# zhiqiangdon/pose-adv-aug

Hardware: AMD Instinct MI355X
Metric: images/sec, 2-stack HG 256x256 bs=24 per GPU, full training step (higher is better)
Workload: dtype bf16; 1 GPU; BASELINE configs[1]: 2-stack hourglass chan 256, bs=24/GPU, 256x256 MPII-shape synthetic frames (720x1280 uint8 resident in HBM), on-device HumanAug warp, heat-map MSE, RMSprop, PCKh; global_batch=24, parallelism=dp1, ranks_seen=1, devices_seen=1

## Files before the change

### pose_adv_aug_amd/csrc/crop_warp.hip

```cpp
#include "pose_ops.h"

#pragma clang fp contract(off)

#define CW_PREC 22

struct CropPlan {
    int wb, hb;
    int case_b;
    int wd, hd;
    int ulx, uly;
    int nw, nh;
    int cw, ch;
    int pad, rot_mode;
    int dx0, dx1, dy0, dy1;
    int sy0, sy1;
    int sx0, sx1;
    int flip;
    float gain[3];
    double m[6];
    double sx, sy;
};

__device__ __forceinline__ int src_byte(unsigned char k, float gain, bool f32) {
    float v = ((float)k / 255.f) * gain;
    v = fminf(fmaxf(v, 0.f), 1.f);
    if (f32) { const float t = v * 255.f; return (int)(t + 0.5f); }
    return (int)((double)v * 255.0 + 0.5);
}

#define CW_ACC 12
#define CW_TAB 768
// ... 40 lines not shown
    if (xmin < 0) xmin = 0;
    int xmax = (int)(t.center + support + 0.5);
    if (xmax > in_size) xmax = in_size;
    t.xmin = xmin; t.n = xmax - xmin;
    double ww = 0.0;
    for (int x = 0; x < t.n; ++x) {
        double v = ((double)(x + xmin) - t.center + 0.5) * t.ss;
        if (v < 0.0) v = -v;
        ww += v < 1.0 ? 1.0 - v : 0.0;
    }
    t.ww = ww;
    return t;
}
__device__ __forceinline__ int tap_coeff(const Taps& t, int x) {
    double v = ((double)(x + t.xmin) - t.center + 0.5) * t.ss;
    if (v < 0.0) v = -v;
    double w = v < 1.0 ? 1.0 - v : 0.0;
    if (t.ww != 0.0) w = w / t.ww;
    return (int)(0.5 + w * (double)(1 << CW_PREC));
}
__device__ __forceinline__ int clip8(int ss) { ss >>= CW_PREC; return ss < 0 ? 0 : (ss > 255 ? 255 : ss); }

#define CW_KMAX 24
#define CW_ENTRY (2 + CW_KMAX)
__device__ __forceinline__ const int* tap_entry(const int* table, int b, int axis, int axis_max, int i) {
    return table + (((size_t)b * 4 + axis) * axis_max + i) * CW_ENTRY;
}

__global__ void crop_plan_kernel(const double* params, const int* sizes, int Hs, int Ws, int B, int res, CropPlan* plans, unsigned* acc) {
    const int b = blockIdx.x * blockDim.x + threadIdx.x;
    if (b >= B) return;
    if (acc)
        for (int i = 0; i < CW_ACC; ++i) acc[(size_t)b * CW_ACC + i] = (i % 6) < 3 ? 255u : 0u;
    const double* p = params + (size_t)b * 8;
    CropPlan P;
    P.wb = sizes ? sizes[2 * b] : Ws; P.hb = sizes ? sizes[2 * b + 1] : Hs;
    P.flip = p[4] != 0.0;
    for (int c = 0; c < 3; ++c) P.gain[c] = (float)p[5 + c];
    float cx = (float)p[0], cy = (float)p[1], s = (float)p[2];
    const double rot = p[3];
    double sf = (double)(s * 200.f) / (double)res;
    P.case_b = sf >= 2.0;
    if (!P.case_b) sf = 1.0;
    P.wd = P.wb; P.hd = P.hb; P.sx = P.sy = 1.0;
    if (P.case_b) {
        const double frac = 1.0 / sf;
// ... 18 lines not shown
    P.ulx = ulx; P.uly = uly; P.nw = brx - ulx; P.nh = bry - uly;
    for (int i = 0; i < 6; ++i) P.m[i] = 0.0;
    if (rot != 0.0) {
        double angle = fmod(rot, 360.0);
        if (angle < 0.0) angle += 360.0;
        if (angle == 0.0) P.rot_mode = 0;
        else if (angle == 180.0) P.rot_mode = 2;
        else if ((angle == 90.0 || angle == 270.0) && P.nw == P.nh) P.rot_mode = angle == 90.0 ? 3 : 4;
        else {
            P.rot_mode = 1;
            const double ar = -(angle * (3.14159265358979323846 / 180.0));
            const double cs = cos(ar), sn = sin(ar);
            const double rcx = (double)P.nw / 2.0, rcy = (double)P.nh / 2.0;
            P.m[0] = cs; P.m[1] = sn; P.m[3] = -sn; P.m[4] = cs;
            P.m[2] = (P.m[0] * (-rcx) + P.m[1] * (-rcy) + 0.0) + rcx;
            P.m[5] = (P.m[3] * (-rcx) + P.m[4] * (-rcy) + 0.0) + rcy;
        }
    }
    P.dx0 = ulx < 0 ? 0 : ulx; P.dx1 = brx < P.wd ? brx : P.wd;
    P.dy0 = uly < 0 ? 0 : uly; P.dy1 = bry < P.hd ? bry : P.hd;
    if (P.dx1 < P.dx0) P.dx1 = P.dx0;
    if (P.dy1 < P.dy0) P.dy1 = P.dy0;
    P.sy0 = 0; P.sy1 = 0; P.sx0 = 0; P.sx1 = 0;
    if (P.case_b && P.dy1 > P.dy0) {
        const Taps t0 = taps_of(P.dy0, P.hb, P.sy), t1 = taps_of(P.dy1 - 1, P.hb, P.sy);
        P.sy0 = t0.xmin; P.sy1 = t1.xmin + t1.n;
    }
    if (P.case_b && P.dx1 > P.dx0) {
        const Taps t0 = taps_of(P.dx0, P.wb, P.sx), t1 = taps_of(P.dx1 - 1, P.wb, P.sx);
        P.sx0 = t0.xmin; P.sx1 = t1.xmin + t1.n;
    }
    plans[b] = P;
}

__global__ void crop_coeff_kernel(const CropPlan* plans, int res, int* table, int axis_max) {
    const CropPlan& P = plans[blockIdx.y];
    const int axis = blockIdx.z;
    int count, first, in_size; double scale;
    if (axis == 0) { if (!P.case_b) return; count = P.dx1 - P.dx0; first = P.dx0; in_size = P.wb; scale = P.sx; }
    else if (axis == 1) { if (!P.case_b) return; count = P.dy1 - P.dy0; first = P.dy0; in_size = P.hb; scale = P.sy; }
    else if (axis == 2) { if (P.cw == res) return; count = res; first = 0; in_size = P.cw; scale = (double)P.cw / (double)res; }
    else { if (P.ch == res) return; count = res; first = 0; in_size = P.ch; scale = (double)P.ch / (double)res; }
    const int i = blockIdx.x * blockDim.x + threadIdx.x;
    if (i >= count || i >= axis_max) return;
    const Taps t = taps_of(first + i, in_size, scale);
    int* e = table + (((size_t)blockIdx.y * 4 + axis) * axis_max + i) * CW_ENTRY;
    e[0] = t.xmin;
    if (t.n > CW_KMAX) { e[1] = -t.n; return; }
    e[1] = t.n;
    for (int k = 0; k < t.n; ++k) e[2 + k] = tap_coeff(t, k);
}

template <bool STRETCH>
__global__ __launch_bounds__(256) void crop_src_kernel(const unsigned char* src, int Hs, int Ws, const CropPlan* plans, uchar4* s4, size_t s4_stride,
                                                       int s4_pitch, const unsigned* acc) {
    const CropPlan& P = plans[blockIdx.y];
    if (!P.case_b) return;
    const int ncol = P.sx1 - P.sx0, nrow = P.sy1 - P.sy0;
    const unsigned char* img = src + (size_t)blockIdx.y * Hs * Ws * 3;
    uchar4* out = s4 + (size_t)blockIdx.y * s4_stride;
    __shared__ unsigned char lut[3][256];
    if (STRETCH) {
        float lo, hi;
        stretch_range(acc + (size_t)blockIdx.y * CW_ACC, acc + (size_t)blockIdx.y * CW_ACC + 3, P.gain, false, false, lo, hi);
        for (int k = threadIdx.x; k < 768; k += blockDim.x) lut[k >> 8][k & 255] = stretch_f32(src_val((unsigned char)(k & 255), P.gain[k >> 8]), lo, hi);
    } else
        for (int k = threadIdx.x; k < 768; k += blockDim.x) lut[k >> 8][k & 255] = (unsigned char)src_byte((unsigned char)(k & 255), P.gain[k >> 8], true);
    __syncthreads();
    if ((Ws & 3) == 0 && ((size_t)src & 3) == 0) {
        const int lo = P.flip ? P.wb - P.sx1 : P.sx0, hi = lo + ncol;
        const int g0 = lo >> 2, ng = ((hi - 1) >> 2) - g0 + 1;
        const unsigned total = (unsigned)ng * (unsigned)nrow;
        for (unsigned i = blockIdx.x * blockDim.x + threadIdx.x; i < total; i += gridDim.x * blockDim.x) {
            const unsigned r = i / (unsigned)ng, g = i - r * (unsigned)ng;
            const int c0 = (g0 + (int)g) << 2;
            const unsigned* w = reinterpret_cast<const unsigned*>(img + ((size_t)(P.sy0 + (int)r) * Ws + c0) * 3);
            const unsigned w0 = w[0], w1 = w[1], w2 = w[2];
            const unsigned char b[12] = {(unsigned char)w0, (unsigned char)(w0 >> 8), (unsigned char)(w0 >> 16), (unsigned char)(w0 >> 24),
                                         (unsigned char)w1, (unsigned char)(w1 >> 8), (unsigned char)(w1 >> 16), (unsigned char)(w1 >> 24),
                                         (unsigned char)w2, (unsigned char)(w2 >> 8), (unsigned char)(w2 >> 16), (unsigned char)(w2 >> 24)};
            uchar4* orow = out + (size_t)r * s4_pitch;
#pragma unroll
            for (int k = 0; k < 4; ++k) {
                const int cs = c0 + k;
                if (cs < lo || cs >= hi) continue;
                const int x = (P.flip ? P.wb - 1 - cs : cs) - P.sx0;
                orow[x] = make_uchar4(lut[0][b[3 * k]], lut[1][b[3 * k + 1]], lut[2][b[3 * k + 2]], 0);
            }
        }
        return;
    }
    const long total = (long)ncol * nrow;
    for (long i = (long)blockIdx.x * blockDim.x + threadIdx.x; i < total; i += (long)gridDim.x * blockDim.x) {
        const int r = (int)(i / ncol), x = (int)(i - (long)r * ncol);
        const int xs = P.sx0 + x;
        const unsigned char* px = img + ((size_t)(P.sy0 + r) * Ws + (P.flip ? P.wb - 1 - xs : xs)) * 3;
        out[(size_t)r * s4_pitch + x] = make_uchar4(lut[0][px[0]], lut[1][px[1]], lut[2][px[2]], 0);
    }
}

#define CW_HREG 12
#define CW_HROWS 16
template <int NT>
__device__ __forceinline__ void down_h_rows(const uchar4* col, int s4_pitch, uchar4* out, int t1_pitch, int xc, int r0, int nrow, const int* e, int n) {
    int w[NT];
#pragma unroll
    for (int k = 0; k < NT; ++k) w[k] = k < n ? e[2 + k] : 0;
#pragma unroll 2
    for (int j = 0; j < CW_HROWS; ++j) {
        const int r = r0 + 4 * j;
        if (r >= nrow) break;
        const uchar4* row = col + (size_t)r * s4_pitch;
        int a0 = 1 << (CW_PREC - 1), a1 = a0, a2 = a0;
#pragma unroll
        for (int k = 0; k < NT; ++k) {
            const uchar4 px = row[k];
            a0 += (int)px.x * w[k]; a1 += (int)px.y * w[k]; a2 += (int)px.z * w[k];
        }
        out[(size_t)r * t1_pitch + xc] = make_uchar4((unsigned char)clip8(a0), (unsigned char)clip8(a1), (unsigned char)clip8(a2), 0);
    }
}

__global__ __launch_bounds__(256) void crop_down_h_kernel(const CropPlan* plans, const int* table, int axis_max, const uchar4* s4, size_t s4_stride,
                                                          int s4_pitch, uchar4* t1, size_t t1_stride, int t1_pitch, int col_blocks) {
    const CropPlan& P = plans[blockIdx.y];
    if (!P.case_b) return;
    const int ncol = P.dx1 - P.dx0, nrow = P.sy1 - P.sy0;
    const int cb = blockIdx.x % col_blocks, rb = blockIdx.x / col_blocks;
    const int xc = cb * 64 + (threadIdx.x & 63);
    const int r0 = rb * (4 * CW_HROWS) + (threadIdx.x >> 6);
    if (xc >= ncol || r0 >= nrow) return;
    const uchar4* in = s4 + (size_t)blockIdx.y * s4_stride;
    uchar4* out = t1 + (size_t)blockIdx.y * t1_stride;
    const int* e = tap_entry(table, blockIdx.y, 0, axis_max, xc);
    const int xmin = e[0], n = e[1];
    if (n >= 0 && n <= CW_HREG) {
        if (n <= 8) down_h_rows<8>(in + (xmin - P.sx0), s4_pitch, out, t1_pitch, xc, r0, nrow, e, n);
        else down_h_rows<CW_HREG>(in + (xmin - P.sx0), s4_pitch, out, t1_pitch, xc, r0, nrow, e, n);
        return;
    }
    for (int j = 0; j < CW_HROWS; ++j) {
        const int r = r0 + 4 * j;
        if (r >= nrow) break;
        int a0 = 1 << (CW_PREC - 1), a1 = a0, a2 = a0;
        if (n >= 0) {
            const uchar4* row = in + (size_t)r * s4_pitch + (xmin - P.sx0);
            for (int k = 0; k < n; ++k) {
                const uchar4 px = row[k];
                const int w = e[2 + k];
                a0 += (int)px.x * w; a1 += (int)px.y * w; a2 += (int)px.z * w;
            }
        } else {
            const Taps t = taps_of(P.dx0 + xc, P.wb, P.sx);
            const uchar4* row = in + (size_t)r * s4_pitch + (t.xmin - P.sx0);
            for (int k = 0; k < t.n; ++k) {
                const uchar4 px = row[k];
                const int w = tap_coeff(t, k);
                a0 += (int)px.x * w; a1 += (int)px.y * w; a2 += (int)px.z * w;
            }
        }
        out[(size_t)r * t1_pitch + xc] = make_uchar4((unsigned char)clip8(a0), (unsigned char)clip8(a1), (unsigned char)clip8(a2), 0);
    }
}

__global__ void crop_down_v_kernel(const CropPlan* plans, const int* table, int axis_max, const uchar4* t1, size_t t1_stride, int t1_pitch,
                                   uchar4* d, size_t d_stride, int d_pitch) {
    const CropPlan& P = plans[blockIdx.y];
    if (!P.case_b) return;
    const int ncol = P.dx1 - P.dx0, nrow = P.dy1 - P.dy0;
    const long total = (long)ncol * nrow;
    const uchar4* in = t1 + (size_t)blockIdx.y * t1_stride;
    uchar4* out = d + (size_t)blockIdx.y * d_stride;
    for (long i = (long)blockIdx.x * blockDim.x + threadIdx.x; i < total; i += (long)gridDim.x * blockDim.x) {
        const int yr = (int)(i / ncol), xc = (int)(i - (long)yr * ncol);
        const int* e = tap_entry(table, blockIdx.y, 1, axis_max, yr);
        int a0 = 1 << (CW_PREC - 1), a1 = a0, a2 = a0;
        if (e[1] >= 0) {
            const int ymin = e[0], n = e[1];
            for (int k = 0; k < n; ++k) {
                const uchar4 px = in[(size_t)(ymin + k - P.sy0) * t1_pitch + xc];
                const int w = e[2 + k];
                a0 += (int)px.x * w; a1 += (int)px.y * w; a2 += (int)px.z * w;
            }
        } else {
            const Taps t = taps_of(P.dy0 + yr, P.hb, P.sy);
            for (int k = 0; k < t.n; ++k) {
                const uchar4 px = in[(size_t)(t.xmin + k - P.sy0) * t1_pitch + xc];
                const int w = tap_coeff(t, k);
                a0 += (int)px.x * w; a1 += (int)px.y * w; a2 += (int)px.z * w;
            }
        }
        out[(size_t)yr * d_pitch + xc] = make_uchar4((unsigned char)clip8(a0), (unsigned char)clip8(a1), (unsigned char)clip8(a2), 0);
    }
}

__device__ __forceinline__ void minmax_commit(unsigned (&mn)[3], unsigned (&mx)[3], unsigned* a) {
    __shared__ unsigned red[6];
    if (threadIdx.x < 6) red[threadIdx.x] = threadIdx.x < 3 ? 255u : 0u;
    __syncthreads();
#pragma unroll
    for (int c = 0; c < 3; ++c)
        for (int o = 32; o > 0; o >>= 1) {
            const unsigned n = (unsigned)__shfl_xor((int)mn[c], o, 64), x = (unsigned)__shfl_xor((int)mx[c], o, 64);
            mn[c] = n < mn[c] ? n : mn[c]; mx[c] = x > mx[c] ? x : mx[c];
        }
    if ((threadIdx.x & 63) == 0)
        for (int c = 0; c < 3; ++c) { atomicMin(&red[c], mn[c]); atomicMax(&red[3 + c], mx[c]); }
    __syncthreads();
    if (threadIdx.x < 3) atomicMin(&a[threadIdx.x], red[threadIdx.x]);
    else if (threadIdx.x < 6) atomicMax(&a[threadIdx.x], red[threadIdx.x]);
}

__global__ __launch_bounds__(256) void crop_minmax_src_kernel(const unsigned char* src, int Hs, int Ws, const CropPlan* plans, unsigned* acc) {
    const CropPlan& P = plans[blockIdx.y];
    int x0 = 0, x1 = P.wb, y0 = 0, y1 = P.hb;
    unsigned* a = acc + (size_t)blockIdx.y * CW_ACC;
// ... 44 lines not shown
    for (unsigned i = blockIdx.x * blockDim.x + threadIdx.x; i < total; i += gridDim.x * blockDim.x) {
        const unsigned yr = i / (unsigned)ncol, xc = i - yr * (unsigned)ncol;
        const uchar4 px = in[(size_t)yr * d_pitch + xc];
        const unsigned v[3] = {px.x, px.y, px.z};
#pragma unroll
        for (int c = 0; c < 3; ++c) { mn[c] = v[c] < mn[c] ? v[c] : mn[c]; mx[c] = v[c] > mx[c] ? v[c] : mx[c]; }
    }
    minmax_commit(mn, mx, acc + (size_t)blockIdx.y * CW_ACC + 6);
}

__global__ __launch_bounds__(256) void crop_stretch_table_kernel(const CropPlan* plans, const unsigned* acc, unsigned char* tabs) {
    const CropPlan& P = plans[blockIdx.x];
    const unsigned* a = acc + (size_t)blockIdx.x * CW_ACC + 6;
    const bool zero = P.ulx < 0 || P.uly < 0 || P.ulx + P.nw > P.wd || P.uly + P.nh > P.hd;
    float lo, hi;
    stretch_range(a, a + 3, P.gain, P.case_b != 0, zero, lo, hi);
    const unsigned char k = (unsigned char)threadIdx.x;
    unsigned char* tab = tabs + (size_t)blockIdx.x * CW_TAB;
    for (int c = 0; c < 3; ++c)
        tab[c * 256 + k] = stretch_f64(P.case_b ? (double)k : (double)src_val(k, P.gain[c]), (double)lo, (double)hi);
}

template <bool STRETCH>
__device__ __forceinline__ void window_px(const CropPlan& P, const unsigned char* img, int Ws, const uchar4* d, int d_pitch, const unsigned char* tab,
                                          int yy, int xx, int (&v)[3]) {
    const int gx = P.ulx + xx, gy = P.uly + yy;
    v[0] = v[1] = v[2] = 0;
    if (gx < 0 || gy < 0 || gx >= P.wd || gy >= P.hd) return;
    if (P.case_b) {
        const uchar4 px = d[(size_t)(gy - P.dy0) * d_pitch + (gx - P.dx0)];
        if (STRETCH) { v[0] = tab[px.x]; v[1] = tab[256 + px.y]; v[2] = tab[512 + px.z]; }
        else { v[0] = px.x; v[1] = px.y; v[2] = px.z; }
    } else {
        const unsigned char* px = img + ((size_t)gy * Ws + (P.flip ? P.wb - 1 - gx : gx)) * 3;
        if (STRETCH) { v[0] = tab[px[0]]; v[1] = tab[256 + px[1]]; v[2] = tab[512 + px[2]]; }
        else { v[0] = src_byte(px[0], P.gain[0], false); v[1] = src_byte(px[1], P.gain[1], false); v[2] = src_byte(px[2], P.gain[2], false); }
    }
}

template <bool STRETCH>
__global__ void crop_rotate_kernel(const unsigned char* src, int Hs, int Ws, const CropPlan* plans, const uchar4* d, size_t d_stride, int d_pitch,
                                   uchar4* u, size_t u_stride, int u_pitch, const unsigned char* tabs) {
    const CropPlan& P = plans[blockIdx.y];
    if (P.rot_mode == 0) return;
    const unsigned char* tab = STRETCH ? tabs + (size_t)blockIdx.y * CW_TAB : nullptr;
    const long total = (long)P.cw * P.ch;
    const unsigned char* img = src + (size_t)blockIdx.y * Hs * Ws * 3;
    const uchar4* dd = d + (size_t)blockIdx.y * d_stride;
    uchar4* out = u + (size_t)blockIdx.y * u_stride;
    for (long i = (long)blockIdx.x * blockDim.x + threadIdx.x; i < total; i += (long)gridDim.x * blockDim.x) {
        const int y = (int)(i / P.cw), x = (int)(i - (long)y * P.cw);
        const int X = x + P.pad, Y = y + P.pad;
        int o[3] = {0, 0, 0};
        if (P.rot_mode == 2) window_px<STRETCH>(P, img, Ws, dd, d_pitch, tab, P.nh - 1 - Y, P.nw - 1 - X, o);
        else if (P.rot_mode == 3) window_px<STRETCH>(P, img, Ws, dd, d_pitch, tab, X, P.nw - 1 - Y, o);
        else if (P.rot_mode == 4) window_px<STRETCH>(P, img, Ws, dd, d_pitch, tab, P.nh - 1 - X, Y, o);
        else {
            const double xc = (double)X + 0.5, yc = (double)Y + 0.5;
            double xin = P.m[0] * xc + P.m[1] * yc + P.m[2];
            double yin = P.m[3] * xc + P.m[4] * yc + P.m[5];
            if (!(xin < 0.0 || xin >= (double)P.nw || yin < 0.0 || yin >= (double)P.nh)) {
                xin -= 0.5; yin -= 0.5;
                const int fx = (int)floor(xin), fy = (int)floor(yin);
                const double ddx = xin - (double)fx, ddy = yin - (double)fy;
                const int x0 = fx < 0 ? 0 : (fx < P.nw ? fx : P.nw - 1), x1 = fx + 1 < 0 ? 0 : (fx + 1 < P.nw ? fx + 1 : P.nw - 1);
                const int y0 = fy < 0 ? 0 : (fy < P.nh ? fy : P.nh - 1);
                int p00[3], p01[3], p10[3], p11[3];
                window_px<STRETCH>(P, img, Ws, dd, d_pitch, tab, y0, x0, p00); window_px<STRETCH>(P, img, Ws, dd, d_pitch, tab, y0, x1, p01);
// ... 4 lines not shown
                    const double v2 = has1 ? (double)p10[c] + (double)(p11[c] - p10[c]) * ddx : v1;
                    o[c] = (int)(unsigned char)(v1 + (v2 - v1) * ddy);
                }
            }
        }
        out[(size_t)y * u_pitch + x] = make_uchar4((unsigned char)o[0], (unsigned char)o[1], (unsigned char)o[2], 0);
    }
}

template <bool STRETCH>
__device__ __forceinline__ void crop_px(const CropPlan& P, const unsigned char* img, int Ws, const uchar4* d, int d_pitch, const unsigned char* tab,
                                        const uchar4* u, int u_pitch, int y, int x, int (&v)[3]) {
    if (P.rot_mode != 0) { const uchar4 px = u[(size_t)y * u_pitch + x]; v[0] = px.x; v[1] = px.y; v[2] = px.z; return; }
    const int off = (P.nw - P.cw) / 2;
    window_px<STRETCH>(P, img, Ws, d, d_pitch, tab, y + off, x + off, v);
}

template <bool STRETCH>
__global__ void crop_resize_h_kernel(const unsigned char* src, int Hs, int Ws, const CropPlan* plans, const uchar4* d, size_t d_stride, int d_pitch,
                                     const uchar4* u, size_t u_stride, int u_pitch, int res, const int* table, int axis_max, uchar4* t2, size_t t2_stride,
                                     const unsigned char* tabs) {
    const CropPlan& P = plans[blockIdx.y];
    if (P.cw == res && P.ch == res) return;
    const unsigned char* tab = STRETCH ? tabs + (size_t)blockIdx.y * CW_TAB : nullptr;
    const long total = (long)P.ch * res;
    const unsigned char* img = src + (size_t)blockIdx.y * Hs * Ws * 3;
    const uchar4* dd = d + (size_t)blockIdx.y * d_stride;
    const uchar4* uu = u + (size_t)blockIdx.y * u_stride;
    uchar4* out = t2 + (size_t)blockIdx.y * t2_stride;
    const double scale = (double)P.cw / (double)res;
    for (long i = (long)blockIdx.x * blockDim.x + threadIdx.x; i < total; i += (long)gridDim.x * blockDim.x) {
        const int y = (int)(i / res), uo = (int)(i - (long)y * res);
        int v[3];
        if (P.cw == res) {
            crop_px<STRETCH>(P, img, Ws, dd, d_pitch, tab, uu, u_pitch, y, uo, v);
        } else {
            const int* e = tap_entry(table, blockIdx.y, 2, axis_max, uo);
            int a0 = 1 << (CW_PREC - 1), a1 = a0, a2 = a0;
            if (e[1] >= 0) {
                const int xmin = e[0], n = e[1];
                for (int k = 0; k < n; ++k) {
                    int px[3];
                    crop_px<STRETCH>(P, img, Ws, dd, d_pitch, tab, uu, u_pitch, y, xmin + k, px);
                    const int w = e[2 + k];
                    a0 += px[0] * w; a1 += px[1] * w; a2 += px[2] * w;
                }
            } else {
                const Taps t = taps_of(uo, P.cw, scale);
                for (int k = 0; k < t.n; ++k) {
                    int px[3];
                    crop_px<STRETCH>(P, img, Ws, dd, d_pitch, tab, uu, u_pitch, y, t.xmin + k, px);
                    const int w = tap_coeff(t, k);
                    a0 += px[0] * w; a1 += px[1] * w; a2 += px[2] * w;
                }
            }
            v[0] = clip8(a0); v[1] = clip8(a1); v[2] = clip8(a2);
        }
        out[(size_t)y * res + uo] = make_uchar4((unsigned char)v[0], (unsigned char)v[1], (unsigned char)v[2], 0);
    }
}

template <bool STRETCH>
__global__ void crop_resize_v_kernel(const unsigned char* src, int Hs, int Ws, const CropPlan* plans, const uchar4* d, size_t d_stride, int d_pitch,
                                     const uchar4* u, size_t u_stride, int u_pitch, const uchar4* t2, size_t t2_stride, int res,
                                     const int* table, int axis_max, bf16* out4, float* outf, unsigned char* out8, const unsigned char* tabs) {
    const CropPlan& P = plans[blockIdx.y];
    const int b = blockIdx.y;
    const unsigned char* tab = STRETCH ? tabs + (size_t)b * CW_TAB : nullptr;
    const long total = (long)res * res;
    const unsigned char* img = src + (size_t)b * Hs * Ws * 3;
    const uchar4* dd = d + (size_t)b * d_stride;
    const uchar4* uu = u + (size_t)b * u_stride;
    const uchar4* tt = t2 + (size_t)b * t2_stride;
    const double scale = (double)P.ch / (double)res;
    for (long i = (long)blockIdx.x * blockDim.x + threadIdx.x; i < total; i += (long)gridDim.x * blockDim.x) {
        const int vo = (int)(i / res), uo = (int)(i - (long)vo * res);
        int v[3];
        if (P.cw == res && P.ch == res) {
            crop_px<STRETCH>(P, img, Ws, dd, d_pitch, tab, uu, u_pitch, vo, uo, v);
        } else if (P.ch == res) {
            const uchar4 px = tt[(size_t)vo * res + uo]; v[0] = px.x; v[1] = px.y; v[2] = px.z;
        } else {
            const int* e = tap_entry(table, b, 3, axis_max, vo);
            int a0 = 1 << (CW_PREC - 1), a1 = a0, a2 = a0;
            if (e[1] >= 0) {
                const int ymin = e[0], n = e[1];
                for (int k = 0; k < n; ++k) {
                    const uchar4 px = tt[(size_t)(ymin + k) * res + uo];
                    const int w = e[2 + k];
                    a0 += (int)px.x * w; a1 += (int)px.y * w; a2 += (int)px.z * w;
                }
            } else {
                const Taps t = taps_of(vo, P.ch, scale);
                for (int k = 0; k < t.n; ++k) {
                    const uchar4 px = tt[(size_t)(t.xmin + k) * res + uo];
                    const int w = tap_coeff(t, k);
                    a0 += (int)px.x * w; a1 += (int)px.y * w; a2 += (int)px.z * w;
                }
            }
            v[0] = clip8(a0); v[1] = clip8(a1); v[2] = clip8(a2);
        }
        const float o0 = (float)v[0] / 255.f, o1 = (float)v[1] / 255.f, o2 = (float)v[2] / 255.f;
        const size_t t = (size_t)b * total + i;
        if (out4) { bf16x4 ob = {(bf16)o0, (bf16)o1, (bf16)o2, (bf16)0.f}; *reinterpret_cast<bf16x4*>(out4 + t * 4) = ob; }
        if (outf) {
            outf[((size_t)b * 3 + 0) * total + i] = o0; outf[((size_t)b * 3 + 1) * total + i] = o1; outf[((size_t)b * 3 + 2) * total + i] = o2;
        }
        if (out8) { out8[t * 3] = (unsigned char)v[0]; out8[t * 3 + 1] = (unsigned char)v[1]; out8[t * 3 + 2] = (unsigned char)v[2]; }
    }
}

struct CropLayout {
    int pad_b, nw_b, cw_max;
    size_t plans, table, s4, t1, d, u, t2, total;
    int axis_max;
    size_t s4_stride, t1_stride, d_stride, u_stride, t2_stride;
    int s4_pitch, t1_pitch, d_pitch, u_pitch;
};

static CropLayout crop_layout(int B, int Hs, int Ws, int res) {
    CropLayout L;
    L.pad_b = (int)ceil((double)res * 0.70710678118654752 - (double)res / 2.0) + 1;
    L.nw_b = res + 2 * L.pad_b;
    L.cw_max = 2 * res + 2;
    auto align = [](size_t v) { return (v + 255) & ~(size_t)255; };
    size_t off = 0;
    L.plans = off; off = align(off + (size_t)B * sizeof(CropPlan));
    L.axis_max = L.nw_b > res ? L.nw_b : res;
    L.table = off; off = align(off + (size_t)B * 4 * L.axis_max * CW_ENTRY * sizeof(int));
    L.s4_pitch = Ws; L.s4_stride = (size_t)Hs * Ws;
    L.s4 = off; off = align(off + ((size_t)B * L.s4_stride + CW_HREG) * 4);
    L.t1_pitch = L.nw_b; L.t1_stride = (size_t)Hs * L.t1_pitch;
    L.t1 = off; off = align(off + (size_t)B * L.t1_stride * 4);
    L.d_pitch = L.nw_b; L.d_stride = (size_t)L.nw_b * L.d_pitch;
    L.d = off; off = align(off + (size_t)B * L.d_stride * 4);
    L.u_pitch = L.cw_max; L.u_stride = (size_t)L.cw_max * L.u_pitch;
    L.u = off; off = align(off + (size_t)B * L.u_stride * 4);
    L.t2_stride = (size_t)L.cw_max * res;
    L.t2 = off; off = align(off + (size_t)B * L.t2_stride * 4);
    L.total = off;
    return L;
}

size_t pa_crop_workspace_size(int B, int Hs, int Ws, int res) { return crop_layout(B, Hs, Ws, res).total; }

struct CropStretchLayout { size_t acc, tabs, total; };
static CropStretchLayout crop_stretch_layout(int B, const CropLayout& L) {
    auto align = [](size_t v) { return (v + 255) & ~(size_t)255; };
    CropStretchLayout S;
    S.acc = L.total;
    S.tabs = align(S.acc + (size_t)B * CW_ACC * sizeof(unsigned));
    S.total = align(S.tabs + (size_t)B * CW_TAB);
    return S;
}
size_t pa_crop_stretch_workspace_size(int B, int Hs, int Ws, int res) { return crop_stretch_layout(B, crop_layout(B, Hs, Ws, res)).total; }

void pa_crop_bytes_bound(int B, int Hs, int Ws, int res, double* rd, double* wr) {
    const CropLayout L = crop_layout(B, Hs, Ws, res);
    const double frame3 = (double)Hs * Ws * 3, frame4 = (double)Hs * Ws * 4, t1 = (double)Hs * L.nw_b * 4, d = (double)L.nw_b * L.nw_b * 4,
                 u = (double)L.cw_max * L.cw_max * 4, t2 = (double)L.cw_max * res * 4, out = (double)res * res * 4 * 2;
    *rd = B * (frame3 + frame4 + t1 + d + u + t2) + (double)B * 4 * L.axis_max * CW_ENTRY * sizeof(int) * 3;
    *wr = B * (frame4 + t1 + d + u + t2 + out) + (double)B * 4 * L.axis_max * CW_ENTRY * sizeof(int);
}

template <bool STRETCH>
static int launch_crop(const unsigned char* src, int Hs, int Ws, const int* sizes, const double* params, int B, int res, void* workspace,
                       bf16* out4, float* outf, unsigned char* out8, hipStream_t st) {
    const CropLayout L = crop_layout(B, Hs, Ws, res);
    const CropStretchLayout S = crop_stretch_layout(B, L);
    char* ws = reinterpret_cast<char*>(workspace);
    CropPlan* plans = reinterpret_cast<CropPlan*>(ws + L.plans);
    int* table = reinterpret_cast<int*>(ws + L.table);
    uchar4* s4 = reinterpret_cast<uchar4*>(ws + L.s4);
    uchar4* t1 = reinterpret_cast<uchar4*>(ws + L.t1);
    uchar4* d = reinterpret_cast<uchar4*>(ws + L.d);
    uchar4* u = reinterpret_cast<uchar4*>(ws + L.u);
    uchar4* t2 = reinterpret_cast<uchar4*>(ws + L.t2);
    unsigned* acc = STRETCH ? reinterpret_cast<unsigned*>(ws + S.acc) : nullptr;
    unsigned char* tabs = STRETCH ? reinterpret_cast<unsigned char*>(ws + S.tabs) : nullptr;
    hipLaunchKernelGGL(crop_plan_kernel, dim3((B + 63) / 64), dim3(64), 0, st, params, sizes, Hs, Ws, B, res, plans, acc);
    const int T = 256;
    auto blocks = [&](long n) { long g = (n + T - 1) / T; return (unsigned)(g < 1 ? 1 : (g > 1024 ? 1024 : g)); };
    hipLaunchKernelGGL(crop_coeff_kernel, dim3((L.axis_max + 63) / 64, B, 4), dim3(64), 0, st, plans, res, table, L.axis_max);
    if (STRETCH) hipLaunchKernelGGL(crop_minmax_src_kernel, dim3(96, B), dim3(T), 0, st, src, Hs, Ws, plans, acc);
    hipLaunchKernelGGL(crop_src_kernel<STRETCH>, dim3(96, B), dim3(T), 0, st, src, Hs, Ws, plans, s4, L.s4_stride, L.s4_pitch, acc);
    const int col_blocks = (L.axis_max + 63) / 64, row_blocks = (Hs + 4 * CW_HROWS - 1) / (4 * CW_HROWS);
    hipLaunchKernelGGL(crop_down_h_kernel, dim3(col_blocks * row_blocks, B), dim3(T), 0, st, plans, table, L.axis_max, s4, L.s4_stride, L.s4_pitch,
                       t1, L.t1_stride, L.t1_pitch, col_blocks);
    hipLaunchKernelGGL(crop_down_v_kernel, dim3(blocks((long)L.nw_b * L.nw_b), B), dim3(T), 0, st, plans, table, L.axis_max, t1, L.t1_stride, L.t1_pitch,
                       d, L.d_stride, L.d_pitch);
    if (STRETCH) {
        hipLaunchKernelGGL(crop_minmax_d_kernel, dim3(blocks((long)L.nw_b * L.nw_b / 4), B), dim3(T), 0, st, plans, d, L.d_stride, L.d_pitch, acc);
        hipLaunchKernelGGL(crop_stretch_table_kernel, dim3(B), dim3(256), 0, st, plans, acc, tabs);
    }
    hipLaunchKernelGGL(crop_rotate_kernel<STRETCH>, dim3(blocks((long)L.cw_max * L.cw_max / 2), B), dim3(T), 0, st, src, Hs, Ws, plans, d, L.d_stride, L.d_pitch,
                       u, L.u_stride, L.u_pitch, tabs);
    hipLaunchKernelGGL(crop_resize_h_kernel<STRETCH>, dim3(blocks((long)L.cw_max * res / 2), B), dim3(T), 0, st, src, Hs, Ws, plans, d, L.d_stride, L.d_pitch,
                       u, L.u_stride, L.u_pitch, res, table, L.axis_max, t2, L.t2_stride, tabs);
    hipLaunchKernelGGL(crop_resize_v_kernel<STRETCH>, dim3(blocks((long)res * res), B), dim3(T), 0, st, src, Hs, Ws, plans, d, L.d_stride, L.d_pitch,
                       u, L.u_stride, L.u_pitch, t2, L.t2_stride, res, table, L.axis_max, out4, outf, out8, tabs);
    return (int)hipGetLastError();
}

int pa_launch_crop(const unsigned char* src, int Hs, int Ws, const int* sizes, const double* params, int B, int res, void* workspace,
                   bf16* out4, float* outf, unsigned char* out8, hipStream_t st) {
    return launch_crop<false>(src, Hs, Ws, sizes, params, B, res, workspace, out4, outf, out8, st);
}
int pa_launch_crop_stretch(const unsigned char* src, int Hs, int Ws, const int* sizes, const double* params, int B, int res, void* workspace,
                           bf16* out4, float* outf, unsigned char* out8, hipStream_t st) {
    return launch_crop<true>(src, Hs, Ws, sizes, params, B, res, workspace, out4, outf, out8, st);
}
```

Baseline: 4201 images/sec.

## Fuse separable downscale passes through LDS tiles and vectorize source crop

Merges the horizontal and vertical downscale kernels into a single kernel that filters rows into a shared-memory tile and then applies vertical taps, removing the t1 intermediate buffer and its HBM round trip. A fallback wide kernel handles large scale factors in chunked passes. The source gather kernel now processes 16 pixels per thread with 16-byte loads and stores, one row group per block. Per-sample gain lookup tables are now built for the non-stretch path too and staged in LDS, replacing per-pixel float conversion. This adds complexity and LDS usage, and risks divergence between the fused and wide paths.

```diff
diff --git a/pose_adv_aug_amd/csrc/crop_warp.hip b/pose_adv_aug_amd/csrc/crop_warp.hip
--- a/pose_adv_aug_amd/csrc/crop_warp.hip
+++ b/pose_adv_aug_amd/csrc/crop_warp.hip
@@ -7,6 +7,7 @@
 struct CropPlan {
     int wb, hb;
     int case_b;
+    int fused;
     int wd, hd;
     int ulx, uly;
     int nw, nh;
@@ -93,6 +94,9 @@
 __device__ __forceinline__ int clip8(int ss) { ss >>= CW_PREC; return ss < 0 ? 0 : (ss > 255 ? 255 : ss); }
 
 #define CW_KMAX 24
+#define CW_HREG 12
+#define CW_FRB 16
+#define CW_FROWS 96
 #define CW_ENTRY (2 + CW_KMAX)
 __device__ __forceinline__ const int* tap_entry(const int* table, int b, int axis, int axis_max, int i) {
     return table + (((size_t)b * 4 + axis) * axis_max + i) * CW_ENTRY;
@@ -157,6 +161,7 @@
     if (P.dx1 < P.dx0) P.dx1 = P.dx0;
     if (P.dy1 < P.dy0) P.dy1 = P.dy0;
     P.sy0 = 0; P.sy1 = 0; P.sx0 = 0; P.sx1 = 0;
+    P.fused = P.case_b && 2.0 * P.sx + 1.0 <= (double)CW_HREG && (double)(CW_FRB + 1) * P.sy + 2.0 <= (double)CW_FROWS;
     if (P.case_b && P.dy1 > P.dy0) {
         const Taps t0 = taps_of(P.dy0, P.hb, P.sy), t1 = taps_of(P.dy1 - 1, P.hb, P.sy);
         P.sy0 = t0.xmin; P.sy1 = t1.xmin + t1.n;
@@ -168,9 +173,12 @@
     plans[b] = P;
 }
 
-__global__ void crop_coeff_kernel(const CropPlan* plans, int res, int* table, int axis_max) {
+__global__ void crop_coeff_kernel(const CropPlan* plans, int res, int* table, int axis_max, unsigned char* tabs) {
     const CropPlan& P = plans[blockIdx.y];
     const int axis = blockIdx.z;
+    if (tabs && !P.case_b && blockIdx.x == 0 && axis < 3)
+        for (int k = threadIdx.x; k < 256; k += blockDim.x)
+            tabs[(size_t)blockIdx.y * CW_TAB + axis * 256 + k] = (unsigned char)src_byte((unsigned char)k, P.gain[axis], false);
     int count, first, in_size; double scale;
     if (axis == 0) { if (!P.case_b) return; count = P.dx1 - P.dx0; first = P.dx0; in_size = P.wb; scale = P.sx; }
     else if (axis == 1) { if (!P.case_b) return; count = P.dy1 - P.dy0; first = P.dy0; in_size = P.hb; scale = P.sy; }
@@ -186,12 +194,14 @@
     for (int k = 0; k < t.n; ++k) e[2 + k] = tap_coeff(t, k);
 }
 
+#define CW_SROWS 16
 template <bool STRETCH>
 __global__ __launch_bounds__(256) void crop_src_kernel(const unsigned char* src, int Hs, int Ws, const CropPlan* plans, uchar4* s4, size_t s4_stride,
                                                        int s4_pitch, const unsigned* acc) {
     const CropPlan& P = plans[blockIdx.y];
     if (!P.case_b) return;
     const int ncol = P.sx1 - P.sx0, nrow = P.sy1 - P.sy0;
+    if ((int)blockIdx.x * CW_SROWS >= nrow || ncol <= 0) return;
     const unsigned char* img = src + (size_t)blockIdx.y * Hs * Ws * 3;
     uchar4* out = s4 + (size_t)blockIdx.y * s4_stride;
     __shared__ unsigned char lut[3][256];
@@ -202,131 +212,184 @@
     } else
         for (int k = threadIdx.x; k < 768; k += blockDim.x) lut[k >> 8][k & 255] = (unsigned char)src_byte((unsigned char)(k & 255), P.gain[k >> 8], true);
     __syncthreads();
-    if ((Ws & 3) == 0 && ((size_t)src & 3) == 0) {
-        const int lo = P.flip ? P.wb - P.sx1 : P.sx0, hi = lo + ncol;
-        const int g0 = lo >> 2, ng = ((hi - 1) >> 2) - g0 + 1;
-        const unsigned total = (unsigned)ng * (unsigned)nrow;
-        for (unsigned i = blockIdx.x * blockDim.x + threadIdx.x; i < total; i += gridDim.x * blockDim.x) {
-            const unsigned r = i / (unsigned)ng, g = i - r * (unsigned)ng;
-            const int c0 = (g0 + (int)g) << 2;
-            const unsigned* w = reinterpret_cast<const unsigned*>(img + ((size_t)(P.sy0 + (int)r) * Ws + c0) * 3);
-            const unsigned w0 = w[0], w1 = w[1], w2 = w[2];
-            const unsigned char b[12] = {(unsigned char)w0, (unsigned char)(w0 >> 8), (unsigned char)(w0 >> 16), (unsigned char)(w0 >> 24),
-                                         (unsigned char)w1, (unsigned char)(w1 >> 8), (unsigned char)(w1 >> 16), (unsigned char)(w1 >> 24),
-                                         (unsigned char)w2, (unsigned char)(w2 >> 8), (unsigned char)(w2 >> 16), (unsigned char)(w2 >> 24)};
-            uchar4* orow = out + (size_t)r * s4_pitch;
-#pragma unroll
-            for (int k = 0; k < 4; ++k) {
-                const int cs = c0 + k;
-                if (cs < lo || cs >= hi) continue;
-                const int x = (P.flip ? P.wb - 1 - cs : cs) - P.sx0;
-                orow[x] = make_uchar4(lut[0][b[3 * k]], lut[1][b[3 * k + 1]], lut[2][b[3 * k + 2]], 0);
-            }
-        }
-        return;
-    }
-    const long total = (long)ncol * nrow;
-    for (long i = (long)blockIdx.x * blockDim.x + threadIdx.x; i < total; i += (long)gridDim.x * blockDim.x) {
-        const int r = (int)(i / ncol), x = (int)(i - (long)r * ncol);
-        const int xs = P.sx0 + x;
-        const unsigned char* px = img + ((size_t)(P.sy0 + r) * Ws + (P.flip ? P.wb - 1 - xs : xs)) * 3;
-        out[(size_t)r * s4_pitch + x] = make_uchar4(lut[0][px[0]], lut[1][px[1]], lut[2][px[2]], 0);
-    }
-}
-
-#define CW_HREG 12
-#define CW_HROWS 16
+    const int r = (int)blockIdx.x * CW_SROWS + (int)(threadIdx.x >> 4);
+    if (r >= nrow) return;
+    const int lo = P.flip ? P.wb - P.sx1 : P.sx0, hi = lo + ncol;
+    const int g0 = lo >> 4, ng = ((hi - 1) >> 4) - g0 + 1;
+    const bool ld4 = (Ws & 3) == 0 && ((size_t)src & 3) == 0, ld16 = (Ws & 15) == 0 && ((size_t)src & 15) == 0;
+    const bool st16 = (Ws & 3) == 0 && ((size_t)s4 & 15) == 0 && (!P.flip || (P.wb & 3) == 0);
+    const unsigned char* irow = img + (size_t)(P.sy0 + r) * Ws * 3;
+    uchar4* orow = out + (size_t)r * s4_pitch;
+    for (int g = (int)(threadIdx.x & 15); g < ng; g += 16) {
+        const int c0 = (g0 + g) << 4;
+        if (ld4 && c0 >= lo && c0 + 16 <= hi) {
+            unsigned dw[12];
+            if (ld16) {
+                const uint4* w = reinterpret_cast<const uint4*>(irow + (size_t)c0 * 3);
+                const uint4 q0 = w[0], q1 = w[1], q2 = w[2];
+                dw[0] = q0.x; dw[1] = q0.y; dw[2] = q0.z; dw[3] = q0.w; dw[4] = q1.x; dw[5] = q1.y; dw[6] = q1.z; dw[7] = q1.w;
+                dw[8] = q2.x; dw[9] = q2.y; dw[10] = q2.z; dw[11] = q2.w;
+            } else {
+                const unsigned* w = reinterpret_cast<const unsigned*>(irow + (size_t)c0 * 3);
+#pragma unroll
+                for (int j = 0; j < 12; ++j) dw[j] = w[j];
+            }
+            unsigned px[16];
+#pragma unroll
+            for (int j = 0; j < 16; ++j) {
+                const unsigned b0 = (dw[(3 * j) >> 2] >> (8 * ((3 * j) & 3))) & 255u, b1 = (dw[(3 * j + 1) >> 2] >> (8 * ((3 * j + 1) & 3))) & 255u,
+                               b2 = (dw[(3 * j + 2) >> 2] >> (8 * ((3 * j + 2) & 3))) & 255u;
+                px[j] = (unsigned)lut[0][b0] | ((unsigned)lut[1][b1] << 8) | ((unsigned)lut[2][b2] << 16);
+            }
+            unsigned* o = reinterpret_cast<unsigned*>(orow + (P.flip ? P.wb - 16 - c0 : c0));
+            if (st16) {
+#pragma unroll
+                for (int q = 0; q < 4; ++q) {
+                    uint4 v;
+                    v.x = P.flip ? px[15 - 4 * q] : px[4 * q];     v.y = P.flip ? px[14 - 4 * q] : px[4 * q + 1];
+                    v.z = P.flip ? px[13 - 4 * q] : px[4 * q + 2]; v.w = P.flip ? px[12 - 4 * q] : px[4 * q + 3];
+                    reinterpret_cast<uint4*>(o)[q] = v;
+                }
+            } else {
+#pragma unroll
+                for (int j = 0; j < 16; ++j) o[j] = P.flip ? px[15 - j] : px[j];
+            }
+        } else {
+            const int a = c0 < lo ? lo : c0, b = c0 + 16 < hi ? c0 + 16 : hi;
+            for (int cs = a; cs < b; ++cs) {
+                const unsigned char* q = irow + (size_t)cs * 3;
+                orow[P.flip ? P.wb - 1 - cs : cs] = make_uchar4(lut[0][q[0]], lut[1][q[1]], lut[2][q[2]], 0);
+            }
+        }
+    }
+}
+
 template <int NT>
-__device__ __forceinline__ void down_h_rows(const uchar4* col, int s4_pitch, uchar4* out, int t1_pitch, int xc, int r0, int nrow, const int* e, int n) {
+__device__ __forceinline__ void fused_h_rows(const uchar4* col, int s4_pitch, uchar4 (*tile)[64], int lane, int slot, int nr, const int* e, int n) {
     int w[NT];
 #pragma unroll
     for (int k = 0; k < NT; ++k) w[k] = k < n ? e[2 + k] : 0;
 #pragma unroll 2
-    for (int j = 0; j < CW_HROWS; ++j) {
-        const int r = r0 + 4 * j;
-        if (r >= nrow) break;
-        const uchar4* row = col + (size_t)r * s4_pitch;
+    for (int j = slot; j < nr; j += 4) {
+        const uchar4* row = col + (size_t)j * s4_pitch;
         int a0 = 1 << (CW_PREC - 1), a1 = a0, a2 = a0;
 #pragma unroll
         for (int k = 0; k < NT; ++k) {
             const uchar4 px = row[k];
-            a0 += (int)px.x * w[k]; a1 += (int)px.y * w[k]; a2 += (int)px.z * w[k];
-        }
-        out[(size_t)r * t1_pitch + xc] = make_uchar4((unsigned char)clip8(a0), (unsigned char)clip8(a1), (unsigned char)clip8(a2), 0);
-    }
-}
-
-__global__ __launch_bounds__(256) void crop_down_h_kernel(const CropPlan* plans, const int* table, int axis_max, const uchar4* s4, size_t s4_stride,
-                                                          int s4_pitch, uchar4* t1, size_t t1_stride, int t1_pitch, int col_blocks) {
-    const CropPlan& P = plans[blockIdx.y];
-    if (!P.case_b) return;
-    const int ncol = P.dx1 - P.dx0, nrow = P.sy1 - P.sy0;
-    const int cb = blockIdx.x % col_blocks, rb = blockIdx.x / col_blocks;
-    const int xc = cb * 64 + (threadIdx.x & 63);
-    const int r0 = rb * (4 * CW_HROWS) + (threadIdx.x >> 6);
-    if (xc >= ncol || r0 >= nrow) return;
+            a0 += __mul24((int)px.x, w[k]); a1 += __mul24((int)px.y, w[k]); a2 += __mul24((int)px.z, w[k]);
+        }
+        tile[j][lane] = make_uchar4((unsigned char)clip8(a0), (unsigned char)clip8(a1), (unsigned char)clip8(a2), 0);
+    }
+}
+
+__device__ __forceinline__ void down_wide(const CropPlan& P, const int* table, int b, int axis_max, const uchar4* in, int s4_pitch, uchar4* out, int d_pitch,
+                                       uchar4 (*tile)[64], int xc, int ncol, int y0, int nb) {
+    const int lane = threadIdx.x & 63, slot = threadIdx.x >> 6;
+    const bool on = xc < ncol;
+    const int* ex = tap_entry(table, b, 0, axis_max, on ? xc : 0);
+    Taps tx, ty;
+    if (on && ex[1] < 0) tx = taps_of(P.dx0 + xc, P.wb, P.sx);
+    for (int sb = 0; sb < nb; sb += 4) {
+        const int last = sb + 3 < nb ? sb + 3 : nb - 1;
+        const int* ef = tap_entry(table, b, 1, axis_max, y0 + sb);
+        const int* el = tap_entry(table, b, 1, axis_max, y0 + last);
+        const int rfirst = ef[0], nr = el[0] + (el[1] < 0 ? -el[1] : el[1]) - rfirst;
+        const int yr = sb + slot;
+        const bool has = on && yr < nb;
+        const int* e = tap_entry(table, b, 1, axis_max, y0 + (has ? yr : sb));
+        const int n = e[1] < 0 ? -e[1] : e[1];
+        if (has && e[1] < 0) ty = taps_of(P.dy0 + y0 + yr, P.hb, P.sy);
+        int a0 = 1 << (CW_PREC - 1), a1 = a0, a2 = a0;
+        for (int c0 = 0; c0 < nr; c0 += CW_FROWS) {
+            const int cn = nr - c0 < CW_FROWS ? nr - c0 : CW_FROWS;
+            if (on) {
+                for (int j = slot; j < cn; j += 4) {
+                    const uchar4* row = in + (size_t)(rfirst - P.sy0 + c0 + j) * s4_pitch;
+                    int h0 = 1 << (CW_PREC - 1), h1 = h0, h2 = h0;
+                    if (ex[1] >= 0) {
+                        const int xmin = ex[0], nx = ex[1];
+                        for (int k = 0; k < nx; ++k) {
+                            const uchar4 px = row[xmin + k];
+                            const int w = ex[2 + k];
+                            h0 += (int)px.x * w; h1 += (int)px.y * w; h2 += (int)px.z * w;
+                        }
+                    } else {
+                        for (int k = 0; k < tx.n; ++k) {
+                            const uchar4 px = row[tx.xmin + k];
+                            const int w = tap_coeff(tx, k);
+                            h0 += (int)px.x * w; h1 += (int)px.y * w; h2 += (int)px.z * w;
+                        }
+                    }
+                    tile[j][lane] = make_uchar4((unsigned char)clip8(h0), (unsigned char)clip8(h1), (unsigned char)clip8(h2), 0);
+                }
+            }
+            __syncthreads();
+            if (has) {
+                const int j0 = e[0] - rfirst - c0;
+                const int k0 = j0 < 0 ? -j0 : 0, k1 = cn - j0 < n ? cn - j0 : n;
+                for (int k = k0; k < k1; ++k) {
+                    const uchar4 px = tile[j0 + k][lane];
+                    const int w = e[1] < 0 ? tap_coeff(ty, k) : e[2 + k];
+                    a0 += (int)px.x * w; a1 += (int)px.y * w; a2 += (int)px.z * w;
+                }
+            }
+            __syncthreads();
+        }
+        if (has) out[(size_t)(y0 + yr) * d_pitch + xc] = make_uchar4((unsigned char)clip8(a0), (unsigned char)clip8(a1), (unsigned char)clip8(a2), 0);
+    }
+}
+
+__global__ __launch_bounds__(256) void crop_down_fused_kernel(const CropPlan* plans, const int* table, int axis_max, const uchar4* s4, size_t s4_stride,
+                                                              int s4_pitch, uchar4* d, size_t d_stride, int d_pitch, int col_blocks) {
+    const CropPlan& P = plans[blockIdx.y];
+    if (!P.fused) return;
+    const int ncol = P.dx1 - P.dx0, nrow = P.dy1 - P.dy0;
+    const int cb = blockIdx.x % col_blocks, y0 = (blockIdx.x / col_blocks) * CW_FRB;
+    if (cb * 64 >= ncol || y0 >= nrow) return;
+    const int nb = nrow - y0 < CW_FRB ? nrow - y0 : CW_FRB;
+    __shared__ uchar4 tile[CW_FROWS][64];
+    const int lane = threadIdx.x & 63, slot = __builtin_amdgcn_readfirstlane(threadIdx.x >> 6);
+    const int xc = cb * 64 + lane;
     const uchar4* in = s4 + (size_t)blockIdx.y * s4_stride;
-    uchar4* out = t1 + (size_t)blockIdx.y * t1_stride;
-    const int* e = tap_entry(table, blockIdx.y, 0, axis_max, xc);
-    const int xmin = e[0], n = e[1];
-    if (n >= 0 && n <= CW_HREG) {
-        if (n <= 8) down_h_rows<8>(in + (xmin - P.sx0), s4_pitch, out, t1_pitch, xc, r0, nrow, e, n);
-        else down_h_rows<CW_HREG>(in + (xmin - P.sx0), s4_pitch, out, t1_pitch, xc, r0, nrow, e, n);
-        return;
-    }
-    for (int j = 0; j < CW_HROWS; ++j) {
-        const int r = r0 + 4 * j;
-        if (r >= nrow) break;
+    uchar4* out = d + (size_t)blockIdx.y * d_stride;
+    const int* ef = tap_entry(table, blockIdx.y, 1, axis_max, y0);
+    const int* el = tap_entry(table, blockIdx.y, 1, axis_max, y0 + nb - 1);
+    const int rfirst = ef[0];
+    int nr = el[0] + el[1] - rfirst;
+    if (nr > CW_FROWS) nr = CW_FROWS;
+    if (xc < ncol) {
+        const int* e = tap_entry(table, blockIdx.y, 0, axis_max, xc);
+        const int xmin = e[0], n = e[1];
+        const uchar4* col = in + (size_t)(rfirst - P.sy0) * s4_pitch + xmin;
+        if (n <= 8) fused_h_rows<8>(col, s4_pitch, tile, lane, slot, nr, e, n);
+        else fused_h_rows<CW_HREG>(col, s4_pitch, tile, lane, slot, nr, e, n);
+    }
+    __syncthreads();
+    if (xc >= ncol) return;
+    for (int yr = slot; yr < nb; yr += 4) {
+        const int* e = tap_entry(table, blockIdx.y, 1, axis_max, y0 + yr);
+        const int j0 = e[0] - rfirst, n = e[1];
         int a0 = 1 << (CW_PREC - 1), a1 = a0, a2 = a0;
-        if (n >= 0) {
-            const uchar4* row = in + (size_t)r * s4_pitch + (xmin - P.sx0);
-            for (int k = 0; k < n; ++k) {
-                const uchar4 px = row[k];
-                const int w = e[2 + k];
-                a0 += (int)px.x * w; a1 += (int)px.y * w; a2 += (int)px.z * w;
-            }
-        } else {
-            const Taps t = taps_of(P.dx0 + xc, P.wb, P.sx);
-            const uchar4* row = in + (size_t)r * s4_pitch + (t.xmin - P.sx0);
-            for (int k = 0; k < t.n; ++k) {
-                const uchar4 px = row[k];
-                const int w = tap_coeff(t, k);
-                a0 += (int)px.x * w; a1 += (int)px.y * w; a2 += (int)px.z * w;
-            }
-        }
-        out[(size_t)r * t1_pitch + xc] = make_uchar4((unsigned char)clip8(a0), (unsigned char)clip8(a1), (unsigned char)clip8(a2), 0);
-    }
-}
-
-__global__ void crop_down_v_kernel(const CropPlan* plans, const int* table, int axis_max, const uchar4* t1, size_t t1_stride, int t1_pitch,
-                                   uchar4* d, size_t d_stride, int d_pitch) {
-    const CropPlan& P = plans[blockIdx.y];
-    if (!P.case_b) return;
+        for (int k = 0; k < n; ++k) {
+            const int j = j0 + k < CW_FROWS ? j0 + k : CW_FROWS - 1;
+            const uchar4 px = tile[j][lane];
+            const int w = e[2 + k];
+            a0 += __mul24((int)px.x, w); a1 += __mul24((int)px.y, w); a2 += __mul24((int)px.z, w);
+        }
+        out[(size_t)(y0 + yr) * d_pitch + xc] = make_uchar4((unsigned char)clip8(a0), (unsigned char)clip8(a1), (unsigned char)clip8(a2), 0);
+    }
+}
+
+__global__ __launch_bounds__(256) void crop_down_wide_kernel(const CropPlan* plans, const int* table, int axis_max, const uchar4* s4, size_t s4_stride,
+                                                             int s4_pitch, uchar4* d, size_t d_stride, int d_pitch, int col_blocks) {
+    const CropPlan& P = plans[blockIdx.y];
+    if (!P.case_b || P.fused) return;
     const int ncol = P.dx1 - P.dx0, nrow = P.dy1 - P.dy0;
-    const long total = (long)ncol * nrow;
-    const uchar4* in = t1 + (size_t)blockIdx.y * t1_stride;
-    uchar4* out = d + (size_t)blockIdx.y * d_stride;
-    for (long i = (long)blockIdx.x * blockDim.x + threadIdx.x; i < total; i += (long)gridDim.x * blockDim.x) {
-        const int yr = (int)(i / ncol), xc = (int)(i - (long)yr * ncol);
-        const int* e = tap_entry(table, blockIdx.y, 1, axis_max, yr);
-        int a0 = 1 << (CW_PREC - 1), a1 = a0, a2 = a0;
-        if (e[1] >= 0) {
-            const int ymin = e[0], n = e[1];
-            for (int k = 0; k < n; ++k) {
-                const uchar4 px = in[(size_t)(ymin + k - P.sy0) * t1_pitch + xc];
-                const int w = e[2 + k];
-                a0 += (int)px.x * w; a1 += (int)px.y * w; a2 += (int)px.z * w;
-            }
-        } else {
-            const Taps t = taps_of(P.dy0 + yr, P.hb, P.sy);
-            for (int k = 0; k < t.n; ++k) {
-                const uchar4 px = in[(size_t)(t.xmin + k - P.sy0) * t1_pitch + xc];
-                const int w = tap_coeff(t, k);
-                a0 += (int)px.x * w; a1 += (int)px.y * w; a2 += (int)px.z * w;
-            }
-        }
-        out[(size_t)yr * d_pitch + xc] = make_uchar4((unsigned char)clip8(a0), (unsigned char)clip8(a1), (unsigned char)clip8(a2), 0);
-    }
+    const int cb = blockIdx.x % col_blocks, y0 = (blockIdx.x / col_blocks) * CW_FRB;
+    if (cb * 64 >= ncol || y0 >= nrow) return;
+    __shared__ uchar4 tile[CW_FROWS][64];
+    down_wide(P, table, blockIdx.y, axis_max, s4 + (size_t)blockIdx.y * s4_stride, s4_pitch, d + (size_t)blockIdx.y * d_stride, d_pitch, tile,
+              cb * 64 + (int)(threadIdx.x & 63), ncol, y0, nrow - y0 < CW_FRB ? nrow - y0 : CW_FRB);
 }
 
 __device__ __forceinline__ void minmax_commit(unsigned (&mn)[3], unsigned (&mx)[3], unsigned* a) {
@@ -417,6 +480,13 @@
 }
 
 template <bool STRETCH>
+__device__ __forceinline__ bool window_has_tab(const CropPlan& P) { return STRETCH || !P.case_b; }
+__device__ __forceinline__ void window_tab(const unsigned char* tabs, int b, unsigned* lds) {
+    const unsigned* t = reinterpret_cast<const unsigned*>(tabs + (size_t)b * CW_TAB);
+    for (int k = threadIdx.x; k < CW_TAB / 4; k += blockDim.x) lds[k] = t[k];
+    __syncthreads();
+}
+template <bool STRETCH>
 __device__ __forceinline__ void window_px(const CropPlan& P, const unsigned char* img, int Ws, const uchar4* d, int d_pitch, const unsigned char* tab,
                                           int yy, int xx, int (&v)[3]) {
     const int gx = P.ulx + xx, gy = P.uly + yy;
@@ -428,8 +498,7 @@
         else { v[0] = px.x; v[1] = px.y; v[2] = px.z; }
     } else {
         const unsigned char* px = img + ((size_t)gy * Ws + (P.flip ? P.wb - 1 - gx : gx)) * 3;
-        if (STRETCH) { v[0] = tab[px[0]]; v[1] = tab[256 + px[1]]; v[2] = tab[512 + px[2]]; }
-        else { v[0] = src_byte(px[0], P.gain[0], false); v[1] = src_byte(px[1], P.gain[1], false); v[2] = src_byte(px[2], P.gain[2], false); }
+        v[0] = tab[px[0]]; v[1] = tab[256 + px[1]]; v[2] = tab[512 + px[2]];
     }
 }
 
@@ -438,7 +507,9 @@
                                    uchar4* u, size_t u_stride, int u_pitch, const unsigned char* tabs) {
     const CropPlan& P = plans[blockIdx.y];
     if (P.rot_mode == 0) return;
-    const unsigned char* tab = STRETCH ? tabs + (size_t)blockIdx.y * CW_TAB : nullptr;
+    __shared__ unsigned tab_lds[CW_TAB / 4];
+    if (window_has_tab<STRETCH>(P)) window_tab(tabs, blockIdx.y, tab_lds);
+    const unsigned char* tab = reinterpret_cast<const unsigned char*>(tab_lds);
     const long total = (long)P.cw * P.ch;
     const unsigned char* img = src + (size_t)blockIdx.y * Hs * Ws * 3;
     const uchar4* dd = d + (size_t)blockIdx.y * d_stride;
@@ -489,7 +560,9 @@
                                      const unsigned char* tabs) {
     const CropPlan& P = plans[blockIdx.y];
     if (P.cw == res && P.ch == res) return;
-    const unsigned char* tab = STRETCH ? tabs + (size_t)blockIdx.y * CW_TAB : nullptr;
+    __shared__ unsigned tab_lds[CW_TAB / 4];
+    if (P.rot_mode == 0 && window_has_tab<STRETCH>(P)) window_tab(tabs, blockIdx.y, tab_lds);
+    const unsigned char* tab = reinterpret_cast<const unsigned char*>(tab_lds);
     const long total = (long)P.ch * res;
     const unsigned char* img = src + (size_t)blockIdx.y * Hs * Ws * 3;
     const uchar4* dd = d + (size_t)blockIdx.y * d_stride;
@@ -533,7 +606,9 @@
                                      const int* table, int axis_max, bf16* out4, float* outf, unsigned char* out8, const unsigned char* tabs) {
     const CropPlan& P = plans[blockIdx.y];
     const int b = blockIdx.y;
-    const unsigned char* tab = STRETCH ? tabs + (size_t)b * CW_TAB : nullptr;
+    __shared__ unsigned tab_lds[CW_TAB / 4];
+    if (P.rot_mode == 0 && P.cw == res && P.ch == res && window_has_tab<STRETCH>(P)) window_tab(tabs, b, tab_lds);
+    const unsigned char* tab = reinterpret_cast<const unsigned char*>(tab_lds);
     const long total = (long)res * res;
     const unsigned char* img = src + (size_t)b * Hs * Ws * 3;
     const uchar4* dd = d + (size_t)b * d_stride;
@@ -579,10 +654,10 @@
 
 struct CropLayout {
     int pad_b, nw_b, cw_max;
-    size_t plans, table, s4, t1, d, u, t2, total;
+    size_t plans, table, s4, d, u, t2, tabs, total;
     int axis_max;
-    size_t s4_stride, t1_stride, d_stride, u_stride, t2_stride;
-    int s4_pitch, t1_pitch, d_pitch, u_pitch;
+    size_t s4_stride, d_stride, u_stride, t2_stride;
+    int s4_pitch, d_pitch, u_pitch;
 };
 
 static CropLayout crop_layout(int B, int Hs, int Ws, int res) {
@@ -597,37 +672,36 @@
     L.table = off; off = align(off + (size_t)B * 4 * L.axis_max * CW_ENTRY * sizeof(int));
     L.s4_pitch = Ws; L.s4_stride = (size_t)Hs * Ws;
     L.s4 = off; off = align(off + ((size_t)B * L.s4_stride + CW_HREG) * 4);
-    L.t1_pitch = L.nw_b; L.t1_stride = (size_t)Hs * L.t1_pitch;
-    L.t1 = off; off = align(off + (size_t)B * L.t1_stride * 4);
     L.d_pitch = L.nw_b; L.d_stride = (size_t)L.nw_b * L.d_pitch;
     L.d = off; off = align(off + (size_t)B * L.d_stride * 4);
     L.u_pitch = L.cw_max; L.u_stride = (size_t)L.cw_max * L.u_pitch;
     L.u = off; off = align(off + (size_t)B * L.u_stride * 4);
     L.t2_stride = (size_t)L.cw_max * res;
     L.t2 = off; off = align(off + (size_t)B * L.t2_stride * 4);
+    L.tabs = off; off = align(off + (size_t)B * CW_TAB);
     L.total = off;
     return L;
 }
 
 size_t pa_crop_workspace_size(int B, int Hs, int Ws, int res) { return crop_layout(B, Hs, Ws, res).total; }
 
-struct CropStretchLayout { size_t acc, tabs, total; };
+struct CropStretchLayout { size_t acc, total; };
 static CropStretchLayout crop_stretch_layout(int B, const CropLayout& L) {
     auto align = [](size_t v) { return (v + 255) & ~(size_t)255; };
     CropStretchLayout S;
     S.acc = L.total;
-    S.tabs = align(S.acc + (size_t)B * CW_ACC * sizeof(unsigned));
-    S.total = align(S.tabs + (size_t)B * CW_TAB);
+    S.total = align(S.acc + (size_t)B * CW_ACC * sizeof(unsigned));
     return S;
 }
 size_t pa_crop_stretch_workspace_size(int B, int Hs, int Ws, int res) { return crop_stretch_layout(B, crop_layout(B, Hs, Ws, res)).total; }
 
 void pa_crop_bytes_bound(int B, int Hs, int Ws, int res, double* rd, double* wr) {
     const CropLayout L = crop_layout(B, Hs, Ws, res);
-    const double frame3 = (double)Hs * Ws * 3, frame4 = (double)Hs * Ws * 4, t1 = (double)Hs * L.nw_b * 4, d = (double)L.nw_b * L.nw_b * 4,
+    const double frame3 = (double)Hs * Ws * 3, frame4 = (double)Hs * Ws * 4, d = (double)L.nw_b * L.nw_b * 4,
                  u = (double)L.cw_max * L.cw_max * 4, t2 = (double)L.cw_max * res * 4, out = (double)res * res * 4 * 2;
-    *rd = B * (frame3 + frame4 + t1 + d + u + t2) + (double)B * 4 * L.axis_max * CW_ENTRY * sizeof(int) * 3;
-    *wr = B * (frame4 + t1 + d + u + t2 + out) + (double)B * 4 * L.axis_max * CW_ENTRY * sizeof(int);
+    *rd = B * (frame3 + frame4 + d + u + t2) + (double)B * 4 * L.axis_max * CW_ENTRY * sizeof(int) * 3
+          + (double)B * CW_TAB * 3;
+    *wr = B * (frame4 + d + u + t2 + out) + (double)B * 4 * L.axis_max * CW_ENTRY * sizeof(int) + (double)B * CW_TAB;
 }
 
 template <bool STRETCH>
@@ -639,23 +713,23 @@
     CropPlan* plans = reinterpret_cast<CropPlan*>(ws + L.plans);
     int* table = reinterpret_cast<int*>(ws + L.table);
     uchar4* s4 = reinterpret_cast<uchar4*>(ws + L.s4);
-    uchar4* t1 = reinterpret_cast<uchar4*>(ws + L.t1);
     uchar4* d = reinterpret_cast<uchar4*>(ws + L.d);
     uchar4* u = reinterpret_cast<uchar4*>(ws + L.u);
     uchar4* t2 = reinterpret_cast<uchar4*>(ws + L.t2);
     unsigned* acc = STRETCH ? reinterpret_cast<unsigned*>(ws + S.acc) : nullptr;
-    unsigned char* tabs = STRETCH ? reinterpret_cast<unsigned char*>(ws + S.tabs) : nullptr;
+    unsigned char* tabs = reinterpret_cast<unsigned char*>(ws + L.tabs);
     hipLaunchKernelGGL(crop_plan_kernel, dim3((B + 63) / 64), dim3(64), 0, st, params, sizes, Hs, Ws, B, res, plans, acc);
     const int T = 256;
     auto blocks = [&](long n) { long g = (n + T - 1) / T; return (unsigned)(g < 1 ? 1 : (g > 1024 ? 1024 : g)); };
-    hipLaunchKernelGGL(crop_coeff_kernel, dim3((L.axis_max + 63) / 64, B, 4), dim3(64), 0, st, plans, res, table, L.axis_max);
+    hipLaunchKernelGGL(crop_coeff_kernel, dim3((L.axis_max + 63) / 64, B, 4), dim3(64), 0, st, plans, res, table, L.axis_max,
+                       STRETCH ? nullptr : tabs);
     if (STRETCH) hipLaunchKernelGGL(crop_minmax_src_kernel, dim3(96, B), dim3(T), 0, st, src, Hs, Ws, plans, acc);
-    hipLaunchKernelGGL(crop_src_kernel<STRETCH>, dim3(96, B), dim3(T), 0, st, src, Hs, Ws, plans, s4, L.s4_stride, L.s4_pitch, acc);
-    const int col_blocks = (L.axis_max + 63) / 64, row_blocks = (Hs + 4 * CW_HROWS - 1) / (4 * CW_HROWS);
-    hipLaunchKernelGGL(crop_down_h_kernel, dim3(col_blocks * row_blocks, B), dim3(T), 0, st, plans, table, L.axis_max, s4, L.s4_stride, L.s4_pitch,
-                       t1, L.t1_stride, L.t1_pitch, col_blocks);
-    hipLaunchKernelGGL(crop_down_v_kernel, dim3(blocks((long)L.nw_b * L.nw_b), B), dim3(T), 0, st, plans, table, L.axis_max, t1, L.t1_stride, L.t1_pitch,
-                       d, L.d_stride, L.d_pitch);
+    hipLaunchKernelGGL(crop_src_kernel<STRETCH>, dim3((Hs + CW_SROWS - 1) / CW_SROWS, B), dim3(T), 0, st, src, Hs, Ws, plans, s4, L.s4_stride, L.s4_pitch, acc);
+    const int col_blocks = (L.axis_max + 63) / 64;
+    hipLaunchKernelGGL(crop_down_fused_kernel, dim3(col_blocks * ((L.nw_b + CW_FRB - 1) / CW_FRB), B), dim3(T), 0, st, plans, table, L.axis_max, s4, L.s4_stride,
+                       L.s4_pitch, d, L.d_stride, L.d_pitch, col_blocks);
+    hipLaunchKernelGGL(crop_down_wide_kernel, dim3(col_blocks * ((L.nw_b + CW_FRB - 1) / CW_FRB), B), dim3(T), 0, st, plans, table, L.axis_max, s4, L.s4_stride,
+                       L.s4_pitch, d, L.d_stride, L.d_pitch, col_blocks);
     if (STRETCH) {
         hipLaunchKernelGGL(crop_minmax_d_kernel, dim3(blocks((long)L.nw_b * L.nw_b / 4), B), dim3(T), 0, st, plans, d, L.d_stride, L.d_pitch, acc);
         hipLaunchKernelGGL(crop_stretch_table_kernel, dim3(B), dim3(256), 0, st, plans, acc, tabs);
```

Result: no change. 4216 images/sec, median of 3 (+0.4%).
